# draenog/nextsimdg

Measured on AMD Instinct MI355X. Metric: element-steps/sec (dynamics+transport), higher is better.
Workload: dtype f64

## Files before the change

nextsimdg_amd/csrc/mevp_fused4.hip:

```cpp
#include "mevp_p2p.h"

namespace nsdg_mevp_detail {

#ifdef NSDG_P2P_SPINSTAT
__device__ unsigned long long nsdg_p2p_spin_dev[4][4];
__device__ unsigned long long nsdg_p2p_phase_dev[4][8];
#define NSDG_SPIN_ARG , unsigned (&spins)[3], unsigned (&phase)[8], unsigned& stamp_last
#define NSDG_SPIN_PASS , spins, phase, stamp_last
#define NSDG_SPIN_COUNT(k, n) spins[k] += (n)
#define NSDG_PHASE(k)                                                   \
    do {                                                                \
        __builtin_amdgcn_sched_barrier(0);                              \
        const unsigned now_ = (unsigned)__builtin_amdgcn_s_memtime();   \
        phase[k] += now_ - stamp_last;                                  \
        stamp_last = now_;                                              \
        __builtin_amdgcn_sched_barrier(0);                              \
    } while (0)
#else
#define NSDG_PHASE(k)
#define NSDG_SPIN_ARG
#define NSDG_SPIN_PASS
#define NSDG_SPIN_COUNT(k, n) (void)(n)
#endif

constexpr int P4_OWNED = 57, P4_LEFT = 4;
constexpr int P4_HAND = 32;
constexpr int P4_SLOT = P4_HAND * 64;
constexpr int P4_HSLOTS = 2;
constexpr int P4_PRING = 7;
constexpr int P4_PSLOT = P2P_PSLOT;
constexpr int P4_CSLOT = 8 * 64;
constexpr int P4_LDS = 3 * P4_HSLOTS * P4_SLOT + P4_PRING * (P4_PSLOT + P4_CSLOT);

struct Fetch {
    double P[9];
    double c[4][6];
    double s11[8], s12[8], s22[8];
    double ub[3], vb[3], um[3], vm[3], ut[3], vt[3];
};

struct Stage {
    int s;
    int nst;
    int first, last;
    int last_prev;
    int last_final;
    int upd0;
};

struct Flags {
    int v[8];
};

__device__ __forceinline__ int ring_slot(int row) { return row % P4_PRING; }
__device__ __forceinline__ void ring_read_c(const double* __restrict__ cring, int row, int lane, double (&c)[4][6])
{
    const double* s = cring + ring_slot(row) * P4_CSLOT + 2 * lane;
#pragma unroll
    for (int n = 0; n < 4; ++n) {
        const double2 t = *reinterpret_cast<const double2*>(s + n * 128);
        c[n][4] = t.x, c[n][5] = t.y;
    }
}
__device__ __forceinline__ void ring_write_c(double* __restrict__ cring, int row, int lane, const double (&c)[4][6])
{
    double* s = cring + ring_slot(row) * P4_CSLOT + 2 * lane;
#pragma unroll
    for (int n = 0; n < 4; ++n)
        *reinterpret_cast<double2*>(s + n * 128) = make_double2(c[n][4], c[n][5]);
}
__device__ __forceinline__ void load_nodal2(const double* __restrict__ packed, long plane, long n, double (&c)[6])
{
    const double* p = packed + nodal_off(n);
#pragma unroll
    for (int k = 0; k < 2; ++k) {
        const double2 t = *reinterpret_cast<const double2*>(p + k * plane);
        c[2 * k] = t.x, c[2 * k + 1] = t.y;
    }
}
__device__ __forceinline__ void load_owned_nodal2(const MarchConst& M, int nrow, double (&c)[4][6], const double* __restrict__ packed)
{
    const long nVn = (long)(2 * nrow) * M.nn + 2 * M.ix;
    load_nodal2(packed, M.nplane, nVn, c[0]);
    load_nodal2(packed, M.nplane, nVn + 1, c[1]);
    load_nodal2(packed, M.nplane, nVn + M.nn, c[2]);
    load_nodal2(packed, M.nplane, nVn + M.nn + 1, c[3]);
}
__device__ __forceinline__ void hand_stress(double* out, const double (&s11)[8], const double (&s12)[8], const double (&s22)[8])
{
#pragma unroll
    for (int k = 0; k < 4; ++k) {
        lds_pair(out, k, s11[2 * k], s11[2 * k + 1]);
        lds_pair(out, 4 + k, s12[2 * k], s12[2 * k + 1]);
        lds_pair(out, 8 + k, s22[2 * k], s22[2 * k + 1]);
    }
}
__device__ __forceinline__ void store_stress(const StressPtrs& S, long ts, const double (&s11)[8], const double (&s12)[8], const double (&s22)[8])
{
    tile_store8_nt<(NSDG_P2P_NT & 2) != 0>(S.o11, ts, s11);
    tile_store8_nt<(NSDG_P2P_NT & 2) != 0>(S.o12, ts, s12);
    tile_store8_nt<(NSDG_P2P_NT & 2) != 0>(S.o22, ts, s22);
}
template <bool FIRST, bool AD, bool LAND>
__device__ __forceinline__ void p2p_row(const MarchConst& M, const Stage& G, int row, Fetch& f, TopCarry& carry, double* __restrict__ lds,
    volatile lds_int* flags, const P2PReport& rep, const StressPtrs& S, const double* __restrict__ u_old, const double* __restrict__ v_old,
    const double* __restrict__ packed, const double* __restrict__ pg, double* __restrict__ u_new, double* __restrict__ v_new NSDG_SPIN_ARG)
{
    const int stage = FIRST ? 0 : G.s;
    const int nrow = min(row + 1, G.last);
    const int ix = M.ix, nn = M.nn;
    double* const ring = lds + 3 * P4_HSLOTS * P4_SLOT;
    double* const cring = ring + P4_PRING * P4_PSLOT;
    auto request_c = [&](int r) {
        if (FIRST)
            load_owned_nodal(M, r, f.c, packed);
        else {
            load_owned_nodal2(M, r, f.c, packed);
            ring_read_c(cring, r, M.lane, f.c);
        }
    };
    const long nVn = (long)(2 * nrow) * nn + 2 * ix;
    double s11[8], s12[8], s22[8], uu[4], vv[4], ul[9], vl[9], un[4], vn[4];
    if (FIRST) {
#pragma unroll
        for (int a = 0; a < 3; ++a) {
            ul[a] = f.ub[a], ul[3 + a] = f.um[a], ul[6 + a] = f.ut[a];
            vl[a] = f.vb[a], vl[3 + a] = f.vm[a], vl[6 + a] = f.vt[a];
        }
        uu[0] = ul[0], uu[1] = ul[1], uu[2] = ul[3], uu[3] = ul[4];
        vv[0] = vl[0], vv[1] = vl[1], vv[2] = vl[3], vv[3] = vl[4];
    } else {
        NSDG_SPIN_COUNT(0, flag_wait(flags, stage - 1, min(row + 1, G.last_prev), rep));
        if (row == G.first) {
            ring_read_P<P4_PRING>(ring, row, M.lane, f.P);
            request_c(row);
        }
        const double* in = lds + ((stage - 1) * P4_HSLOTS + (row & 1)) * P4_SLOT + 2 * M.lane;
        const double* top = lds + ((stage - 1) * P4_HSLOTS + ((row + 1) & 1)) * P4_SLOT + 2 * M.lane;
#pragma unroll
        for (int k = 0; k < 2; ++k) {
            const double2 a = lds_pair(in, 12 + k), b = lds_pair(in, 14 + k);
            uu[2 * k] = a.x, uu[2 * k + 1] = a.y, vv[2 * k] = b.x, vv[2 * k + 1] = b.y;
        }
        double2 tu = lds_pair(top, 12), tv = lds_pair(top, 14);
        if (row + 1 > G.last_prev)
            tu = tv = make_double2(0., 0.);
        gather_nodes(M, uu, tu.x, tu.y, ul);
        gather_nodes(M, vv, tv.x, tv.y, vl);
    }
    NSDG_PHASE(0);
    double r11[8], r12[8], r22[8];
    double qe = 0., ialpha = M.ialpha;
    if constexpr (AD)
        stress_projected_adaptive(ul, vl, f.P, M.ihx, M.ihy, M.dmin2, f.c[3][0], M.AC, r11, r12, r22, qe, ialpha);
    else
        stress_projected(ul, vl, f.P, M.ihx, M.ihy, M.ialpha, M.dmin2, r11, r12, r22);
    __builtin_amdgcn_sched_barrier(0);
    NSDG_PHASE(1);
    if (FIRST) {
        NSDG_SPIN_COUNT(2, flag_wait(flags, 3 + G.nst - 2, min(row - P4_PRING, G.last_final), rep));
        ring_write_P<P4_PRING>(ring, row, M.lane, f.P);
        ring_write_c(cring, row, M.lane, f.c);
        tile_load9_nt<(NSDG_P2P_NT & 4) != 0>(pg, tile_off(ix, nrow, M.ntx, 9), ix & 63, f.P);
        if (nrow > row) {
#pragma unroll
            for (int a = 0; a < 3; ++a)
                f.ub[a] = f.ut[a], f.vb[a] = f.vt[a];
        }
        fetch_nodes(u_old, nVn + nn, f.um);
        fetch_nodes(v_old, nVn + nn, f.vm);
        fetch_nodes(u_old, nVn + 2 * nn, f.ut);
        fetch_nodes(v_old, nVn + 2 * nn, f.vt);
#pragma unroll
        for (int i = 0; i < 8; ++i)
            s11[i] = f.s11[i], s12[i] = f.s12[i], s22[i] = f.s22[i];
    } else {
        ring_read_P<P4_PRING>(ring, nrow, M.lane, f.P);
        const double* in = lds + ((stage - 1) * P4_HSLOTS + (row & 1)) * P4_SLOT + 2 * M.lane;
#pragma unroll
        for (int k = 0; k < 4; ++k) {
            const double2 a = lds_pair(in, k), b = lds_pair(in, 4 + k), c = lds_pair(in, 8 + k);
            s11[2 * k] = a.x, s11[2 * k + 1] = a.y, s12[2 * k] = b.x, s12[2 * k + 1] = b.y, s22[2 * k] = c.x, s22[2 * k + 1] = c.y;
        }
        flag_publish(flags, 3 + stage - 1, row);
    }
    NSDG_PHASE(2);
    stress_relax(ialpha, r11, r12, r22, s11, s12, s22);
    __builtin_amdgcn_sched_barrier(0);
    if (FIRST) {
        const long ts = tile_off(ix, nrow, M.ntx, 8);
        tile_load8_nt<(NSDG_P2P_NT & 1) != 0>(S.i11, ts, f.s11);
        tile_load8_nt<(NSDG_P2P_NT & 1) != 0>(S.i12, ts, f.s12);
        tile_load8_nt<(NSDG_P2P_NT & 1) != 0>(S.i22, ts, f.s22);
    }
    constexpr bool EARLY_HAND = (NSDG_P2P_EARLY & 1) != 0, EARLY_STORE = (NSDG_P2P_EARLY & 2) != 0;
    if constexpr (EARLY_HAND) {
        if (FIRST || stage < G.nst - 1) {
            NSDG_SPIN_COUNT(1, flag_wait(flags, 3 + stage, row - P4_HSLOTS, rep));
            hand_stress(lds + (stage * P4_HSLOTS + (row & 1)) * P4_SLOT + 2 * M.lane, s11, s12, s22);
        }
    }
    if constexpr (EARLY_STORE) {
        if (!(FIRST || stage < G.nst - 1) && M.own && row >= M.y0)
            store_stress(S, tile_off(ix, row, M.ntx, 8), s11, s12, s22);
    }
    NSDG_PHASE(3);
    {
        double cx[9], cy[9];
        node_contrib_all(s11, s12, s22, M.hx, M.hy, cx, cy);
        owned_node_updates<AD, LAND>(M, row > 0, f.c, uu, vv, carry, cx, cy, un, vn, qe);
        if (row < G.upd0) {
#pragma unroll
            for (int k = 0; k < 4; ++k)
                un[k] = vn[k] = 0.;
        }
        carry_top<AD>(carry, cx, cy, qe);
    }
    __builtin_amdgcn_sched_barrier(0);
    NSDG_PHASE(4);
    request_c(nrow);
    NSDG_PHASE(5);
    if (FIRST || stage < G.nst - 1) {
        if constexpr (!EARLY_HAND)
            NSDG_SPIN_COUNT(1, flag_wait(flags, 3 + stage, row - P4_HSLOTS, rep));
        double* out = lds + (stage * P4_HSLOTS + (row & 1)) * P4_SLOT + 2 * M.lane;
        if constexpr (!EARLY_HAND)
            hand_stress(out, s11, s12, s22);
#pragma unroll
        for (int k = 0; k < 2; ++k) {
            lds_pair(out, 12 + k, un[2 * k], un[2 * k + 1]);
            lds_pair(out, 14 + k, vn[2 * k], vn[2 * k + 1]);
        }
        flag_publish(flags, stage, row);
    } else if (M.own && row >= M.y0) {
        const long ts = tile_off(ix, row, M.ntx, 8);
        const long nV = (long)(2 * row) * nn + 2 * ix;
        if constexpr (!EARLY_STORE)
            store_stress(S, ts, s11, s12, s22);
        store_owned_nodes(nV, nn, M.lastcol, row == M.ny - 1, un, vn, u_new, v_new);
    }
    NSDG_PHASE(6);
}

template <bool AD, bool LAND>
__global__ __launch_bounds__(256) void mevp_fused4_kernel(NodalConsts K, AdaptConsts AC, int nst, int nx, int ny, int j0, int j1, int j0b, int j1b, int nsA, int R, int ncw,
    double hx, double hy, double ialpha, double dmin2, P2PReport rep, StressPtrs S, const double* __restrict__ u_old, const double* __restrict__ v_old,
    const double* __restrict__ packed, const double* __restrict__ pg, double* __restrict__ u_new, double* __restrict__ v_new)
{
    __shared__ __attribute__((aligned(16))) double lds[P4_LDS];
    __shared__ Flags flagmem;
    volatile lds_int* flags = (volatile lds_int*)flagmem.v;
    const int lane = threadIdx.x & 63;
    const int group = xcd_contiguous_block(blockIdx.x, gridDim.x);
    int strip = group / ncw;
    const int cw = group - strip * ncw;
    if (strip >= nsA) {
        strip -= nsA;
        j0 = j0b, j1 = j1b;
    }
    MarchConst M;
    M.y0 = j0 + strip * R;
    if (M.y0 >= j1)
        return;
    M.y1 = min(M.y0 + R, j1);
    march_frame<P4_OWNED, P4_LEFT>(M, K, AC, nx, ny, lane, cw, hx, hy, ialpha, dmin2);

    Stage G;
    G.s = __builtin_amdgcn_readfirstlane(threadIdx.x >> 6);
    G.nst = nst;
    auto first_of = [&](int s) { return max(M.y0 - nst + s, 0); };
    auto last_of = [&](int s) { return min(M.y1 + nst - 2 - s, ny - 1); };
    G.first = first_of(G.s);
    G.last = last_of(G.s);
    G.last_prev = last_of(G.s - 1);
    G.last_final = last_of(nst - 1);
    G.upd0 = G.s == 0 ? 0 : M.y0 - (nst - 1) + G.s;

    if (threadIdx.x < 3) {
        flags[threadIdx.x] = first_of(threadIdx.x) - 1;
        flags[3 + threadIdx.x] = first_of(threadIdx.x + 1) - 1;
    }
    if (threadIdx.x == P2P_GIVEUP)
        flags[P2P_GIVEUP] = 0;
    __syncthreads();
    if (G.s >= nst)
        return;

    Fetch f;
    TopCarry carry;
#ifdef NSDG_P2P_SPINSTAT
    unsigned spins[3] = { 0, 0, 0 }, phase[8] = { 0, 0, 0, 0, 0, 0, 0, 0 };
    unsigned stamp_last = (unsigned)__builtin_amdgcn_s_memtime();
#endif
    if (G.s == 0) {
        const int row = G.first;
        const long nV = (long)(2 * row) * M.nn + 2 * M.ix, ts = tile_off(M.ix, row, M.ntx, 8);
        fetch_nodes(u_old, nV, f.ub);
        fetch_nodes(v_old, nV, f.vb);
        fetch_nodes(u_old, nV + M.nn, f.um);
        fetch_nodes(v_old, nV + M.nn, f.vm);
        fetch_nodes(u_old, nV + 2 * M.nn, f.ut);
        fetch_nodes(v_old, nV + 2 * M.nn, f.vt);
        tile_load8_nt<(NSDG_P2P_NT & 1) != 0>(S.i11, ts, f.s11);
        tile_load8_nt<(NSDG_P2P_NT & 1) != 0>(S.i12, ts, f.s12);
        tile_load8_nt<(NSDG_P2P_NT & 1) != 0>(S.i22, ts, f.s22);
        tile_load9_nt<(NSDG_P2P_NT & 4) != 0>(pg, tile_off(M.ix, row, M.ntx, 9), M.ix & 63, f.P);
        load_owned_nodal(M, row, f.c, packed);
        for (int row = G.first; row <= G.last; ++row)
            p2p_row<true, AD, LAND>(M, G, row, f, carry, lds, flags, rep, S, u_old, v_old, packed, pg, u_new, v_new NSDG_SPIN_PASS);
    } else {
        for (int row = G.first; row <= G.last; ++row)
            p2p_row<false, AD, LAND>(M, G, row, f, carry, lds, flags, rep, S, u_old, v_old, packed, pg, u_new, v_new NSDG_SPIN_PASS);
    }
#ifdef NSDG_P2P_SPINSTAT
    if (lane == 0) {
        for (int k = 0; k < 3; ++k)
            atomicAdd(&nsdg_p2p_spin_dev[G.s][k], (unsigned long long)spins[k]);
        atomicAdd(&nsdg_p2p_spin_dev[G.s][3], (unsigned long long)(G.last - G.first + 1));
        for (int k = 0; k < 8; ++k)
            atomicAdd(&nsdg_p2p_phase_dev[G.s][k], (unsigned long long)phase[k]);
    }
#endif
}

}

using namespace nsdg_mevp_detail;

#ifdef NSDG_P2P_SPINSTAT
extern "C" int nsdg_debug_p2p_spinstat(unsigned long long* out48)
{
    static const unsigned long long zero[32] = { 0 };
    hipError_t e = hipMemcpyFromSymbol(out48, HIP_SYMBOL(nsdg_p2p_spin_dev), 16 * sizeof(unsigned long long));
    if (e == hipSuccess)
        e = hipMemcpyFromSymbol(out48 + 16, HIP_SYMBOL(nsdg_p2p_phase_dev), 32 * sizeof(unsigned long long));
    if (e == hipSuccess)
        e = hipMemcpyToSymbol(HIP_SYMBOL(nsdg_p2p_spin_dev), zero, 16 * sizeof(unsigned long long));
    if (e == hipSuccess)
        e = hipMemcpyToSymbol(HIP_SYMBOL(nsdg_p2p_phase_dev), zero, 32 * sizeof(unsigned long long));
    return (int)e;
}
#endif

int nsdg_launch_mevp_fused4_ranges(nsdg_ctx* ctx, bool land, int nst, int j0, int j1, int j0b, int j1b, const nsdg_mevp_bufs& b)
{
    const int ncw = nsdg_div_up(ctx->nx, P4_OWNED);
    const int rowsB = j0b < j1b ? j1b - j0b : 0;
    int R = ctx->strip_rows;
    if (R <= 0) {
        const double extra = 4. * nst - 3.;
        const long slots = ctx->num_cus;
        double best = 1e30;
        R = 64;
        for (int r = 1; r <= 4096; ++r) {
            const long groups = ((long)nsdg_div_up(j1 - j0, r) + nsdg_div_up(rowsB, r)) * ncw;
            const long rounds = (groups + slots - 1) / slots;
            const double cost = rounds * (r + extra);
            if (cost < best) {
                best = cost;
                R = r;
            }
            if (groups <= ncw * (rowsB ? 2 : 1))
                break;
        }
    }
    const int nsA = nsdg_div_up(j1 - j0, R), nsB = nsdg_div_up(rowsB, R);
    const long ngroups = (long)ncw * (nsA + nsB);
    const StressPtrs S = { b.s11i, b.s12i, b.s22i, b.s11, b.s12, b.s22 };
    const NodalConsts K = nsdg_nodal_consts(ctx);
    const AdaptConsts AC = nsdg_adapt_consts(ctx);
    const P2PReport rep = { ctx->p2p_count_dev, ctx->p2p_flag_dev };
    auto launch = [&](auto kernel) {
        hipLaunchKernelGGL(kernel, dim3(ngroups), dim3(256), 0, ctx->stream, K, AC, nst, ctx->nx, ctx->ny, j0, j1, j0b, j1b, nsA, R, ncw, ctx->hx, ctx->hy,
            1. / ctx->mevp.alpha, ctx->mevp.delta_min * ctx->mevp.delta_min, rep, S, b.u_old, b.v_old, b.packed, b.pg, b.u_new, b.v_new);
    };
    if (!land)
        nsdg_adaptive(ctx) ? launch(mevp_fused4_kernel<true, false>) : launch(mevp_fused4_kernel<false, false>);
    else
        nsdg_adaptive(ctx) ? launch(mevp_fused4_kernel<true, true>) : launch(mevp_fused4_kernel<false, true>);
    NSDG_CHECK_LAUNCH();
    return NSDG_OK;
}
```

nextsimdg_amd/csrc/mevp_p2p.h:

```cpp
#pragma once
#include "mevp_pipeline.h"

namespace nsdg_mevp_detail {

#ifndef NSDG_P2P_SPIN_LIMIT
#define NSDG_P2P_SPIN_LIMIT (1 << 20)
#endif

struct P2PReport {
    unsigned* count;
    unsigned* flag;
};

constexpr int P2P_GIVEUP = 6;

typedef __attribute__((address_space(3))) int lds_int;
__device__ __forceinline__ int flag_peek(const volatile lds_int* p)
{
    asm volatile("" ::: "memory");
    const int x = *p;
    asm volatile("" ::: "memory");
    return __builtin_amdgcn_readfirstlane(x);
}
__device__ __forceinline__ int flag_wait(volatile lds_int* flags, int which, int need, const P2PReport& rep)
{
    if (flag_peek(flags + which) >= need)
        return 0;
    for (int spin = 0; spin < NSDG_P2P_SPIN_LIMIT; ++spin) {
        __builtin_amdgcn_s_sleep(1);
        if (flag_peek(flags + which) >= need || flag_peek(flags + P2P_GIVEUP) != 0)
            return spin + 1;
    }
    flags[P2P_GIVEUP] = 1;
    if ((threadIdx.x & 63) == 0) {
        atomicAdd(rep.count, 1u);
        __hip_atomic_store(rep.flag, 1u, __ATOMIC_RELAXED, __HIP_MEMORY_SCOPE_SYSTEM);
    }
    return NSDG_P2P_SPIN_LIMIT;
}
__device__ __forceinline__ void flag_publish(volatile lds_int* flags, int which, int value)
{
    asm volatile("s_waitcnt lgkmcnt(0)" ::: "memory");
    flags[which] = value;
    asm volatile("" ::: "memory");
}

__device__ __forceinline__ double2 lds_pair(const double* slot, int k) { return *reinterpret_cast<const double2*>(slot + k * 128); }
__device__ __forceinline__ void lds_pair(double* slot, int k, double a, double b) { *reinterpret_cast<double2*>(slot + k * 128) = make_double2(a, b); }

#ifndef NSDG_P2P_NT
#define NSDG_P2P_NT 3
#endif
#ifndef NSDG_P2P_EARLY
#define NSDG_P2P_EARLY 2
#endif
typedef double nsdg_pair16 __attribute__((ext_vector_type(2)));
template <bool NT>
__device__ __forceinline__ void tile_load8_nt(const double* __restrict__ a, long t, double (&c)[8])
{
    if (!NT)
        return tile_load8(a, t, c);
#pragma unroll
    for (int k = 0; k < 4; ++k) {
        const nsdg_pair16 v = __builtin_nontemporal_load(reinterpret_cast<const nsdg_pair16*>(a + t + 128 * k));
        c[2 * k] = v.x, c[2 * k + 1] = v.y;
    }
}
template <bool NT>
__device__ __forceinline__ void tile_load9_nt(const double* __restrict__ a, long t, int l, double (&c)[9])
{
    if (!NT)
        return tile_load9(a, t, l, c);
#pragma unroll
    for (int k = 0; k < 4; ++k) {
        const nsdg_pair16 v = __builtin_nontemporal_load(reinterpret_cast<const nsdg_pair16*>(a + t + 128 * k));
        c[2 * k] = v.x, c[2 * k + 1] = v.y;
    }
    c[8] = __builtin_nontemporal_load(a + t + 512 - l);
}
template <bool NT>
__device__ __forceinline__ void tile_store8_nt(double* __restrict__ a, long t, const double (&c)[8])
{
    if (!NT)
        return tile_store8(a, t, c);
#pragma unroll
    for (int k = 0; k < 4; ++k) {
        nsdg_pair16 v;
        v.x = c[2 * k], v.y = c[2 * k + 1];
        __builtin_nontemporal_store(v, reinterpret_cast<nsdg_pair16*>(a + t + 128 * k));
    }
}
typedef double nsdg_pair8 __attribute__((ext_vector_type(2), aligned(8)));
__device__ __forceinline__ void fetch_nodes(const double* __restrict__ w, long n, double (&o)[3])
{
    const nsdg_pair8 a = *reinterpret_cast<const nsdg_pair8*>(w + n);
    o[0] = a.x, o[1] = a.y, o[2] = w[n + 2];
}

constexpr int P2P_PSLOT = 9 * 64;
template <int NR>
__device__ __forceinline__ void ring_read_P(const double* __restrict__ ring, int row, int lane, double (&P)[9])
{
    const double* s = ring + (row % NR) * P2P_PSLOT;
#pragma unroll
    for (int k = 0; k < 4; ++k) {
        const double2 t = *reinterpret_cast<const double2*>(s + k * 128 + 2 * lane);
        P[2 * k] = t.x, P[2 * k + 1] = t.y;
    }
    P[8] = s[512 + lane];
}
template <int NR>
__device__ __forceinline__ void ring_write_P(double* __restrict__ ring, int row, int lane, const double (&P)[9])
{
    double* s = ring + (row % NR) * P2P_PSLOT;
#pragma unroll
    for (int k = 0; k < 4; ++k)
        *reinterpret_cast<double2*>(s + k * 128 + 2 * lane) = make_double2(P[2 * k], P[2 * k + 1]);
    s[512 + lane] = P[8];
}

}
```

Measured before the change: 147.2 million.

## Land prefetched loads with explicit vmcnt waits and defer stress prefetch

Adds explicit s_waitcnt vmcnt landing points with register-pinning asm so the compiler cannot insert conservative full waits on prefetched coefficient, velocity and stress registers. The coefficient ring write is moved after a partial vmcnt wait. The next row's stress tile load is moved to after the halo publish, so more loads stay in flight across the compute. It also adds optional SPINSTAT timing probes. The hand-tuned vmcnt counts depend on the exact order in which loads are issued, and a wrong count could read data before it has arrived.

```diff
diff --git a/nextsimdg_amd/csrc/mevp_fused4.hip b/nextsimdg_amd/csrc/mevp_fused4.hip
--- a/nextsimdg_amd/csrc/mevp_fused4.hip
+++ b/nextsimdg_amd/csrc/mevp_fused4.hip
@@ -5,9 +5,13 @@
 #ifdef NSDG_P2P_SPINSTAT
 __device__ unsigned long long nsdg_p2p_spin_dev[4][4];
 __device__ unsigned long long nsdg_p2p_phase_dev[4][8];
-#define NSDG_SPIN_ARG , unsigned (&spins)[3], unsigned (&phase)[8], unsigned& stamp_last
-#define NSDG_SPIN_PASS , spins, phase, stamp_last
+__device__ unsigned long long nsdg_p2p_land_dev[4];
+#define NSDG_SPIN_ARG , unsigned (&spins)[3], unsigned (&phase)[8], unsigned& stamp_last, unsigned (&landc)[4]
+#define NSDG_SPIN_PASS , spins, phase, stamp_last, landc
 #define NSDG_SPIN_COUNT(k, n) spins[k] += (n)
+#if NSDG_P2P_SPINSTAT + 0 == 2
+#define NSDG_PHASE(k)
+#else
 #define NSDG_PHASE(k)                                                   \
     do {                                                                \
         __builtin_amdgcn_sched_barrier(0);                              \
@@ -16,11 +20,24 @@
         stamp_last = now_;                                              \
         __builtin_amdgcn_sched_barrier(0);                              \
     } while (0)
+#endif
+#define NSDG_LAND_TIMED(k, ...)                                                     \
+    do {                                                                            \
+        const unsigned land0_ = (unsigned)__builtin_amdgcn_s_memtime();             \
+        __VA_ARGS__;                                                                \
+        landc[k] += (unsigned)__builtin_amdgcn_s_memtime() - land0_;                \
+    } while (0)
 #else
 #define NSDG_PHASE(k)
 #define NSDG_SPIN_ARG
 #define NSDG_SPIN_PASS
 #define NSDG_SPIN_COUNT(k, n) (void)(n)
+#define NSDG_LAND_TIMED(k, ...) __VA_ARGS__
+#endif
+#if defined(NSDG_P2P_SPINSTAT) && NSDG_P2P_LAND == 0
+#define NSDG_LAND_PROBE(k, n) NSDG_LAND_TIMED(k, p2p_wait_vm<n>())
+#else
+#define NSDG_LAND_PROBE(k, n)
 #endif
 
 constexpr int P4_OWNED = 57, P4_LEFT = 4;
@@ -100,6 +117,15 @@
     tile_store8_nt<(NSDG_P2P_NT & 2) != 0>(S.o11, ts, s11);
     tile_store8_nt<(NSDG_P2P_NT & 2) != 0>(S.o12, ts, s12);
     tile_store8_nt<(NSDG_P2P_NT & 2) != 0>(S.o22, ts, s22);
+}
+constexpr int P4_NA = 5, P4_NB = 8, P4_NC = 12;
+constexpr bool P4_LAND_COEFF = (NSDG_P2P_LAND & 1) != 0, P4_LAND_ORDER = (NSDG_P2P_LAND & 2) != 0;
+constexpr int P4_L1 = P4_LAND_ORDER ? P4_NC + P4_NA + P4_NB : P4_NA + P4_NB;
+__device__ __forceinline__ void request_stress(const StressPtrs& S, long ts, Fetch& f)
+{
+    tile_load8_nt<(NSDG_P2P_NT & 1) != 0>(S.i11, ts, f.s11);
+    tile_load8_nt<(NSDG_P2P_NT & 1) != 0>(S.i12, ts, f.s12);
+    tile_load8_nt<(NSDG_P2P_NT & 1) != 0>(S.i22, ts, f.s22);
 }
 template <bool FIRST, bool AD, bool LAND>
 __device__ __forceinline__ void p2p_row(const MarchConst& M, const Stage& G, int row, Fetch& f, TopCarry& carry, double* __restrict__ lds,
@@ -122,6 +148,7 @@
     const long nVn = (long)(2 * nrow) * nn + 2 * ix;
     double s11[8], s12[8], s22[8], uu[4], vv[4], ul[9], vl[9], un[4], vn[4];
     if (FIRST) {
+        NSDG_LAND_PROBE(0, 12);
 #pragma unroll
         for (int a = 0; a < 3; ++a) {
             ul[a] = f.ub[a], ul[3 + a] = f.um[a], ul[6 + a] = f.ut[a];
@@ -160,8 +187,15 @@
     if (FIRST) {
         NSDG_SPIN_COUNT(2, flag_wait(flags, 3 + G.nst - 2, min(row - P4_PRING, G.last_final), rep));
         ring_write_P<P4_PRING>(ring, row, M.lane, f.P);
+#if defined(NSDG_P2P_SPINSTAT) && NSDG_P2P_LAND == 0
+        tile_load9_nt<(NSDG_P2P_NT & 4) != 0>(pg, tile_off(ix, nrow, M.ntx, 9), ix & 63, f.P);
+        NSDG_LAND_PROBE(1, P4_NA);
         ring_write_c(cring, row, M.lane, f.c);
+#else
+        if constexpr (!P4_LAND_COEFF)
+            ring_write_c(cring, row, M.lane, f.c);
         tile_load9_nt<(NSDG_P2P_NT & 4) != 0>(pg, tile_off(ix, nrow, M.ntx, 9), ix & 63, f.P);
+#endif
         if (nrow > row) {
 #pragma unroll
             for (int a = 0; a < 3; ++a)
@@ -171,9 +205,11 @@
         fetch_nodes(v_old, nVn + nn, f.vm);
         fetch_nodes(u_old, nVn + 2 * nn, f.ut);
         fetch_nodes(v_old, nVn + 2 * nn, f.vt);
-#pragma unroll
-        for (int i = 0; i < 8; ++i)
-            s11[i] = f.s11[i], s12[i] = f.s12[i], s22[i] = f.s22[i];
+        if constexpr (!P4_LAND_ORDER) {
+#pragma unroll
+            for (int i = 0; i < 8; ++i)
+                s11[i] = f.s11[i], s12[i] = f.s12[i], s22[i] = f.s22[i];
+        }
     } else {
         ring_read_P<P4_PRING>(ring, nrow, M.lane, f.P);
         const double* in = lds + ((stage - 1) * P4_HSLOTS + (row & 1)) * P4_SLOT + 2 * M.lane;
@@ -185,9 +221,19 @@
         flag_publish(flags, 3 + stage - 1, row);
     }
     NSDG_PHASE(2);
+    if constexpr (FIRST && P4_LAND_COEFF) {
+        p2p_name(r11), p2p_name(r12), p2p_name(r22);
+        NSDG_LAND_TIMED(1, p2p_land<P4_L1>(f.c));
+        ring_write_c(cring, row, M.lane, f.c);
+    }
+    if constexpr (FIRST && P4_LAND_ORDER) {
+#pragma unroll
+        for (int i = 0; i < 8; ++i)
+            s11[i] = f.s11[i], s12[i] = f.s12[i], s22[i] = f.s22[i];
+    }
     stress_relax(ialpha, r11, r12, r22, s11, s12, s22);
     __builtin_amdgcn_sched_barrier(0);
-    if (FIRST) {
+    if (FIRST && !P4_LAND_ORDER) {
         const long ts = tile_off(ix, nrow, M.ntx, 8);
         tile_load8_nt<(NSDG_P2P_NT & 1) != 0>(S.i11, ts, f.s11);
         tile_load8_nt<(NSDG_P2P_NT & 1) != 0>(S.i12, ts, f.s12);
@@ -218,6 +264,9 @@
     }
     __builtin_amdgcn_sched_barrier(0);
     NSDG_PHASE(4);
+    if (FIRST) {
+        NSDG_LAND_PROBE(3, 4);
+    }
     request_c(nrow);
     NSDG_PHASE(5);
     if (FIRST || stage < G.nst - 1) {
@@ -232,6 +281,8 @@
             lds_pair(out, 14 + k, vn[2 * k], vn[2 * k + 1]);
         }
         flag_publish(flags, stage, row);
+        if constexpr (FIRST && P4_LAND_ORDER)
+            request_stress(S, tile_off(ix, nrow, M.ntx, 8), f);
     } else if (M.own && row >= M.y0) {
         const long ts = tile_off(ix, row, M.ntx, 8);
         const long nV = (long)(2 * row) * nn + 2 * ix;
@@ -291,6 +342,7 @@
 #ifdef NSDG_P2P_SPINSTAT
     unsigned spins[3] = { 0, 0, 0 }, phase[8] = { 0, 0, 0, 0, 0, 0, 0, 0 };
     unsigned stamp_last = (unsigned)__builtin_amdgcn_s_memtime();
+    unsigned landc[4] = { 0, 0, 0, 0 };
 #endif
     if (G.s == 0) {
         const int row = G.first;
@@ -306,6 +358,12 @@
         tile_load8_nt<(NSDG_P2P_NT & 1) != 0>(S.i22, ts, f.s22);
         tile_load9_nt<(NSDG_P2P_NT & 4) != 0>(pg, tile_off(M.ix, row, M.ntx, 9), M.ix & 63, f.P);
         load_owned_nodal(M, row, f.c, packed);
+        if constexpr (NSDG_P2P_LAND != 0) {
+            p2p_land<0>(f.P, f.ub, f.vb, f.um, f.vm, f.ut, f.vt, f.s11, f.s12, f.s22, f.c);
+#pragma unroll
+            for (int n = 0; n < 4; ++n)
+                p2p_name(f.c[n][0], f.c[n][1], f.c[n][2], f.c[n][3]);
+        }
         for (int row = G.first; row <= G.last; ++row)
             p2p_row<true, AD, LAND>(M, G, row, f, carry, lds, flags, rep, S, u_old, v_old, packed, pg, u_new, v_new NSDG_SPIN_PASS);
     } else {
@@ -319,6 +377,9 @@
         atomicAdd(&nsdg_p2p_spin_dev[G.s][3], (unsigned long long)(G.last - G.first + 1));
         for (int k = 0; k < 8; ++k)
             atomicAdd(&nsdg_p2p_phase_dev[G.s][k], (unsigned long long)phase[k]);
+        if (G.s == 0)
+            for (int k = 0; k < 4; ++k)
+                atomicAdd(&nsdg_p2p_land_dev[k], (unsigned long long)landc[k]);
     }
 #endif
 }
@@ -338,6 +399,14 @@
         e = hipMemcpyToSymbol(HIP_SYMBOL(nsdg_p2p_spin_dev), zero, 16 * sizeof(unsigned long long));
     if (e == hipSuccess)
         e = hipMemcpyToSymbol(HIP_SYMBOL(nsdg_p2p_phase_dev), zero, 32 * sizeof(unsigned long long));
+    return (int)e;
+}
+extern "C" int nsdg_debug_p2p_landstat(unsigned long long* out4)
+{
+    static const unsigned long long zero[4] = { 0 };
+    hipError_t e = hipMemcpyFromSymbol(out4, HIP_SYMBOL(nsdg_p2p_land_dev), 4 * sizeof(unsigned long long));
+    if (e == hipSuccess)
+        e = hipMemcpyToSymbol(HIP_SYMBOL(nsdg_p2p_land_dev), zero, 4 * sizeof(unsigned long long));
     return (int)e;
 }
 #endif
diff --git a/nextsimdg_amd/csrc/mevp_p2p.h b/nextsimdg_amd/csrc/mevp_p2p.h
--- a/nextsimdg_amd/csrc/mevp_p2p.h
+++ b/nextsimdg_amd/csrc/mevp_p2p.h
@@ -54,6 +54,32 @@
 #ifndef NSDG_P2P_EARLY
 #define NSDG_P2P_EARLY 2
 #endif
+#ifndef NSDG_P2P_LAND
+#define NSDG_P2P_LAND 3
+#endif
+template <int N>
+__device__ __forceinline__ void p2p_wait_vm()
+{
+    static_assert(N >= 0 && N < 64, "vmcnt is a 6-bit field");
+    asm volatile("s_waitcnt vmcnt(%0)" ::"n"(N) : "memory");
+}
+__device__ __forceinline__ void p2p_name(double& a, double& b, double& c, double& d) { asm volatile("" : "+v"(a), "+v"(b), "+v"(c), "+v"(d)); }
+__device__ __forceinline__ void p2p_name(double& a, double& b, double& c) { asm volatile("" : "+v"(a), "+v"(b), "+v"(c)); }
+__device__ __forceinline__ void p2p_name(double& a) { asm volatile("" : "+v"(a)); }
+__device__ __forceinline__ void p2p_name(double (&x)[3]) { p2p_name(x[0], x[1], x[2]); }
+__device__ __forceinline__ void p2p_name(double (&x)[8]) { p2p_name(x[0], x[1], x[2], x[3]), p2p_name(x[4], x[5], x[6], x[7]); }
+__device__ __forceinline__ void p2p_name(double (&x)[9]) { p2p_name(x[0], x[1], x[2], x[3]), p2p_name(x[4], x[5], x[6], x[7]), p2p_name(x[8]); }
+__device__ __forceinline__ void p2p_name(double (&c)[4][6])
+{
+    p2p_name(c[0][4], c[0][5], c[1][4], c[1][5]), p2p_name(c[2][4], c[2][5], c[3][4], c[3][5]);
+}
+template <int N, class... T>
+__device__ __forceinline__ void p2p_land(T&... x)
+{
+    p2p_wait_vm<N>();
+    (p2p_name(x), ...);
+}
+
 typedef double nsdg_pair16 __attribute__((ext_vector_type(2)));
 template <bool NT>
 __device__ __forceinline__ void tile_load8_nt(const double* __restrict__ a, long t, double (&c)[8])
```

Result: faster. 152.6 million, median of 6 (+3.7%).
